# beilsme/rs-image-segmentation

Measured on AMD Instinct MI355X. Metric: Mpixel/s feature-extract+classify, higher is better.
Workload: dtype f32

## Files before the change

include/rsseg.h:

```cpp
#ifndef RSSEG_H
#define RSSEG_H

#include <stddef.h>
#include <stdint.h>

#ifdef __cplusplus
extern "C" {
#endif

#define RSSEG_OK 0
#define RSSEG_ERR_INVALID (-1)
#define RSSEG_ERR_HIP (-2)
#define RSSEG_ERR_NOMEM (-3)
#define RSSEG_ERR_COMM (-4)
#define RSSEG_ERR_UNSUPPORTED (-5)

#define RSSEG_F32 0
#define RSSEG_F64 1
#define RSSEG_I64 2
#define RSSEG_U8 3
#define RSSEG_I16 4
#define RSSEG_U16 5
#define RSSEG_I32 6

// ... 110 lines not shown
#define RSSEG_MORPH_GRADIENT 4
int rsseg_morph_u8(rsseg_ctx *ctx, const uint8_t *d_q, int H, int W, int k, int op, uint8_t *d_out);
int rsseg_morph_rows_u8(rsseg_ctx *ctx, const uint8_t *d_q, int Hin, int W, int y0, int y1, int edges, int k, int op,
                        uint8_t *d_out);
int rsseg_laplacian_norm_u8(rsseg_ctx *ctx, const uint8_t *d_q, int H, int W, float *d_out);
int rsseg_laplacian_norm_rows_u8(rsseg_ctx *ctx, const uint8_t *d_q, int Hin, int W, int y0, int y1, int edges, float *d_out);
int rsseg_sobel_mag_u8(rsseg_ctx *ctx, const uint8_t *d_q, int H, int W, float *d_out);
int rsseg_sobel_mag_rows_u8(rsseg_ctx *ctx, const uint8_t *d_q, int Hin, int W, int y0, int y1, int edges, float *d_out);

typedef struct rsseg_kmeans_info {
    int32_t n_iter;
    int32_t relocated;
    double tol;
    double scale[RSSEG_MAX_FEATURES];
    double min[RSSEG_MAX_FEATURES];
    double mean[RSSEG_MAX_FEATURES];
    int64_t init_indices[RSSEG_MAX_CLUSTERS];
    double ms_init;
    double ms_lloyd;
} rsseg_kmeans_info;

int rsseg_kmeans_fit_predict(rsseg_ctx *ctx, const void *const *d_planes, int F, int dtype, int64_t n_local,
                             int k, uint32_t seed, int max_iter, double tol, int32_t *d_labels,
                             double *centers, rsseg_kmeans_info *info);
int rsseg_kmeans_fit_predict_mm(rsseg_ctx *ctx, const void *const *d_planes, int F, int dtype, int64_t n_local, int k,
                                uint32_t seed, int max_iter, double tol, int32_t *d_labels, double *centers,
                                rsseg_kmeans_info *info, const double *local_min, const double *local_max);

int rsseg_forest_load(rsseg_ctx *ctx, int n_trees, const int64_t *tree_off, const int32_t *left,
                      const int32_t *right, const int32_t *feature, const double *threshold,
                      const uint8_t *missing_go_left, const double *value, int n_classes,
                      const int64_t *classes, int n_features);
int rsseg_forest_predict(rsseg_ctx *ctx, const float *const *d_planes, int F, int64_t n, int64_t *d_out);
int rsseg_forest_predict_proba(rsseg_ctx *ctx, const float *const *d_planes, int F, int64_t n, double *d_proba, double *d_conf,
                               int64_t *d_labels);
int rsseg_forest_oob(rsseg_ctx *ctx, const float *const *d_planes, int F, int64_t n, const int32_t *d_counts, double *d_oob,
                     int32_t *d_n_oob);

int rsseg_forest_fit(rsseg_ctx *ctx, const float *const *d_planes, int F, int64_t n, const int32_t *d_y, int n_classes,
                     const int32_t *d_counts, int same_counts, int n_trees, const uint32_t *seeds, int max_depth,
                     int min_samples_split, int min_samples_leaf, int max_features, const int64_t *node_off,
                     int32_t *d_left, int32_t *d_right, int32_t *d_feature, double *d_threshold, double *d_impurity,
                     int32_t *d_n_node, int32_t *d_w_node, uint8_t *d_missing_left, double *d_value,
                     int64_t *node_count, int32_t *max_depth_out);
typedef struct rsseg_forest_job {
    int64_t counts_row;
    int64_t weight_total;
    uint32_t seed;
    int32_t max_depth, min_samples_split, min_samples_leaf, max_features;
    int32_t reserved;
} rsseg_forest_job;
int rsseg_forest_fit_jobs(rsseg_ctx *ctx, const float *const *d_planes, int F, int64_t n, const int32_t *d_y, int n_classes,
                          const int32_t *d_counts, int64_t n_count_rows, int n_trees, const rsseg_forest_job *jobs,
                          const int64_t *node_off, int32_t *d_left, int32_t *d_right, int32_t *d_feature, double *d_threshold,
                          double *d_impurity, int32_t *d_n_node, int32_t *d_w_node, uint8_t *d_missing_left, double *d_value,
                          int64_t *node_count, int32_t *max_depth_out);

int rsseg_threshold_band_f32(rsseg_ctx *ctx, const float *d_x, int64_t n, float lo, float hi, uint8_t *d_out);
int rsseg_band_interval_f32(rsseg_ctx *ctx, const float *d_x, int64_t n, float lo, float hi, int nan_as_zero, uint8_t *d_out);
int rsseg_band_interval_f64(rsseg_ctx *ctx, const double *d_x, int64_t n, double lo, double hi, int nan_as_zero, uint8_t *d_out);
int rsseg_otsu_mask(rsseg_ctx *ctx, const void *d_x, int dtype, int64_t n, int above, uint8_t *d_out, int *level, double *vmin,
                    double *vmax);
int rsseg_mask_op_u8(rsseg_ctx *ctx, const uint8_t *d_a, const uint8_t *d_b, int64_t n, int op, uint8_t *d_out);
int rsseg_mask_paint_u8(rsseg_ctx *ctx, uint8_t *d_map, const uint8_t *d_mask, int64_t n, int value, int only_unset);
int rsseg_morph_ellipse_u8(rsseg_ctx *ctx, const uint8_t *d_q, int H, int W, int k, int op, uint8_t *d_out);
int rsseg_remove_small_components_u8(rsseg_ctx *ctx, const uint8_t *d_mask, int H, int W, int min_area, uint8_t *d_out);
// ... 23 lines not shown
```

rs-image-segmentation_amd/csrc/common.h:

```cpp
#pragma once
#include <hip/hip_runtime.h>
#include <stdint.h>
#include <stdio.h>
#include <string.h>

#include <map>
#include <string>
#include <vector>

#include "../../include/rsseg.h"

#define WAVE 64

struct prof_entry {
    double ms = 0.0;
    int64_t launches = 0;
    std::vector<std::pair<hipEvent_t, hipEvent_t>> pending;
};

struct forest_dev {
    void *d_nodes = nullptr;
    void *d_leafval = nullptr;
    void *d_treeoff = nullptr;
    void *d_groups = nullptr;
    int n_groups = 0;
    int n_trees = 0, n_classes = 0, n_features = 0, max_depth = 0;
    int64_t n_nodes = 0;
    int64_t classes[64];
};

struct rsseg_ctx {
    int device = 0;
    hipStream_t stream = nullptr;
    bool own_stream = false;
    bool async_mode = false;
    char err[512] = {0};
    int rank = 0, world = 1;
    std::vector<std::pair<const void *, int64_t>> byte_valued;
    bool comm_on = false;
    rsseg_allreduce_fn allreduce = nullptr;
    void *comm_user = nullptr;
    char *d_comm = nullptr;
    size_t comm_bytes = 0;
    char *h_comm = nullptr;
    void *rccl_comm = nullptr;
    bool own_comm_buf = false;
    char *d_ws = nullptr;
    size_t ws_bytes = 0;
    char *h_pin = nullptr;
    size_t pin_bytes = 0;
    bool prof_on = false;
    std::map<std::string, prof_entry> prof;
    std::vector<hipEvent_t> event_pool;
    forest_dev forest;
    bool mm_collect = false;
    uint32_t *d_mm = nullptr;
    int mm_count = 0;
// ... 196 lines not shown
```

rs-image-segmentation_amd/csrc/ctx.hip:

```cpp
#include <dlfcn.h>
#include <stdarg.h>

#include <chrono>
#include <mutex>

#include "common.h"

int rs_fail(rsseg_ctx *ctx, int code, const char *fmt, ...)
{
    if (ctx) {
        va_list ap;
        va_start(ap, fmt);
        vsnprintf(ctx->err, sizeof(ctx->err), fmt, ap);
        va_end(ap);
    }
    return code;
}

static thread_local char g_err[256] = "no context";

extern "C" const char *rsseg_version(void) { return "rsseg-hip 0.1 (gfx950)"; }

extern "C" const char *rsseg_last_error(const rsseg_ctx *ctx) { return ctx ? ctx->err : g_err; }

// ... 157 lines not shown
    ctx->world = world;
    ctx->allreduce = rccl_allreduce;
    ctx->comm_user = ctx;
    ctx->comm_on = true;
    if (hipHostMalloc((void **)&ctx->h_comm, comm_bytes, hipHostMallocDefault) != hipSuccess) {
        rccl_release(ctx);
        ctx->comm_on = false;
        ctx->allreduce = nullptr;
        return rs_fail(ctx, RSSEG_ERR_NOMEM, "hipHostMalloc(%zu) for the communication staging buffer failed", comm_bytes);
    }
    return RSSEG_OK;
}

extern "C" void rsseg_ctx_destroy(rsseg_ctx *ctx)
{
    if (!ctx) return;
    (void)hipSetDevice(ctx->device);
    (void)hipStreamSynchronize(ctx->stream);
    for (auto &kv : ctx->prof)
        for (auto &p : kv.second.pending) {
            (void)hipEventDestroy(p.first);
            (void)hipEventDestroy(p.second);
        }
    for (auto ev : ctx->event_pool) (void)hipEventDestroy(ev);
    if (ctx->d_ws) (void)hipFree(ctx->d_ws);
    if (ctx->h_pin) (void)hipHostFree(ctx->h_pin);
    if (ctx->h_comm) (void)hipHostFree(ctx->h_comm);
    rccl_release(ctx);
    if (ctx->d_mm) (void)hipFree(ctx->d_mm);
    if (ctx->forest.d_nodes) (void)hipFree(ctx->forest.d_nodes);
    if (ctx->forest.d_leafval) (void)hipFree(ctx->forest.d_leafval);
    if (ctx->forest.d_treeoff) (void)hipFree(ctx->forest.d_treeoff);
    if (ctx->forest.d_groups) (void)hipFree(ctx->forest.d_groups);
    if (ctx->own_stream) (void)hipStreamDestroy(ctx->stream);
    delete ctx;
}

extern "C" int rsseg_ctx_set_comm(rsseg_ctx *ctx, int rank, int world, rsseg_allreduce_fn fn, void *user,
                                  void *d_comm, size_t comm_bytes)
{
    if (!ctx) return RSSEG_ERR_INVALID;
    rccl_release(ctx);
    if (world < 1 || rank < 0 || rank >= world || world > RSSEG_MAX_RANKS)
        return rs_fail(ctx, RSSEG_ERR_INVALID, "bad rank/world %d/%d", rank, world);
    if (world > 1 && (!fn || !d_comm || comm_bytes < (1u << 20)))
        return rs_fail(ctx, RSSEG_ERR_INVALID, "world > 1 needs an all-reduce hook and a >= 1 MiB comm buffer");
    ctx->rank = rank;
    ctx->world = world;
    ctx->allreduce = fn;
    ctx->comm_user = user;
    ctx->d_comm = (char *)d_comm;
    ctx->comm_bytes = comm_bytes;
    ctx->comm_on = world > 1 || (fn && d_comm && comm_bytes >= (1u << 20));
    if (ctx->h_comm) (void)hipHostFree(ctx->h_comm);
    ctx->h_comm = nullptr;
    if (ctx->comm_on) {
        HIPCHK(ctx, hipSetDevice(ctx->device));
        if (hipHostMalloc((void **)&ctx->h_comm, comm_bytes, hipHostMallocDefault) != hipSuccess)
            return rs_fail(ctx, RSSEG_ERR_NOMEM, "hipHostMalloc(%zu) for the communication staging buffer failed", comm_bytes);
    }
    return RSSEG_OK;
}

static int comm_hook(rsseg_ctx *ctx, int64_t offset, int64_t count, int dtype, int op)
{
    const int rc = ctx->allreduce(ctx->comm_user, offset, count, dtype, op);
// ... 376 lines not shown
```

rs-image-segmentation_amd/csrc/k11_forest.h:

```cpp
#pragma once
#include <algorithm>

#include "common.h"

struct __align__(8) rf_node {
    float thr;
    unsigned bits;
};
#define RF_LEAF 0x00800000u
#define RF_MISS 0x00400000u
#define RF_CHILD 0x003fffffu
#define RF_NAN_BITS 0x7fc00000u
#define RF_PAY_MASK 0x003fffffu

#define RF_NCMAX 64
static_assert(RSSEG_MAX_FEATURES <= 64, "byte 3 of a node holds 4 * feature");
#define RF_C 4

struct rf_planes {
    const float *p[RSSEG_MAX_FEATURES];
};

struct rf_tree {
    int node_off;
// ... 6 lines not shown
    int first, count;
    int node_base;
    int n_nodes;
};

typedef __attribute__((address_space(3))) const float lds_cfloat;
typedef __attribute__((address_space(3))) const rf_node lds_cnode;
#if defined(__HIP_DEVICE_COMPILE__)
#define RF_LDS_PTR(T, a) ((T *)(a))
#else
#define RF_LDS_PTR(T, a) ((T *)(uintptr_t)(a))
#endif

template <int NC>
__device__ __forceinline__ void rf_row_load(const rf_node nd, const double *__restrict__ leafval, double (&row)[NC])
{
    const double2 *v = reinterpret_cast<const double2 *>(leafval + (size_t)(__float_as_uint(nd.thr) & RF_PAY_MASK) * NC);
#pragma unroll
    for (int c = 0; c < NC / 2; c++) {
        const double2 t = v[c];
        row[2 * c] = t.x;
        row[2 * c + 1] = t.y;
    }
}
template <int NC>
__device__ __forceinline__ void rf_vote(const rf_node nd, const double *__restrict__ leafval, double (&acc)[NC])
{
    double row[NC];
    rf_row_load<NC>(nd, leafval, row);
#pragma unroll
    for (int c = 0; c < NC; c++) acc[c] += row[c];
}


template <int TH>
__device__ __forceinline__ int rf_stage_features(const rf_planes &pl, int F, int64_t n, int64_t i, float *feat)
{
    int my_nan = 0;
    for (int f = 0; f < F; f++) {
        const float v = i < n ? pl.p[f][i] : 0.f;
        my_nan |= v != v;
        feat[f * TH + threadIdx.x] = v;
    }
    return my_nan;
}

#define RF_PX 1
#define RF_NCH (RF_PX * RF_C)

template <bool NANS>
__device__ __forceinline__ void rf_round_lds(rf_node (&nd)[RF_NCH], unsigned feat_tid, unsigned px_stride, const unsigned (&base)[RF_C])
{
    float x[RF_NCH];
#pragma unroll
    for (int q = 0; q < RF_NCH; q++)
        x[q] = *RF_LDS_PTR(lds_cfloat, feat_tid + (q / RF_C) * px_stride + (nd[q].bits >> 24));
#pragma unroll
    for (int q = 0; q < RF_NCH; q++) {
        bool go_right = x[q] > nd[q].thr;
        if (NANS) go_right = go_right || (x[q] != x[q] && !(nd[q].bits & RF_MISS));
        const unsigned next = (nd[q].bits & RF_CHILD) + (go_right ? 1u : 0u);
        lds_cnode *p = RF_LDS_PTR(lds_cnode, base[q % RF_C] + next * 8u);
        nd[q].thr = p->thr;
        nd[q].bits = p->bits;
    }
}
// ... 68 lines not shown
```

rs-image-segmentation_amd/csrc/k11_forest.hip:

```cpp
#include <algorithm>
#include <cmath>
#include <queue>

#include "common.h"
#include "k11_forest.h"

template <int NC>
__device__ __forceinline__ void rf_finish(const double (&acc)[NC], int n_trees, int n_classes, const long long *__restrict__ classes,
                                          long long *__restrict__ out, int64_t i)
{
    int best = 0;
    double bv = acc[0] / (double)n_trees;
#pragma unroll
    for (int c = 1; c < NC; c++)
        if (c < n_classes) {
            const double p = acc[c] / (double)n_trees;
            if (p > bv) { bv = p; best = c; }
        }
    out[i] = classes[best];
}

template <int NC, int RF_TH>
__global__ __launch_bounds__(RF_TH) void k11_forest_lds(rf_planes pl, int F, int64_t n, const rf_node *__restrict__ nodes,
                                                        const rf_tree *__restrict__ trees, const rf_group *__restrict__ groups, int n_groups,
                                                        int cap2 , int two_rounds, int n_trees,
                                                        const double *__restrict__ leafval,
                                                        int n_classes, const long long *__restrict__ classes, long long *__restrict__ out)
{
    constexpr int RF_LT = RF_TH / RF_PX;
    extern __shared__ __align__(16) char smem[];
    const int FP = F | 1;
    float *feat = reinterpret_cast<float *>(smem);
    uint4 *top = reinterpret_cast<uint4 *>(feat + (size_t)FP * RF_TH);
    const int64_t i0 = (int64_t)blockIdx.x * RF_TH + threadIdx.x;
    int my_nan = 0;
    for (int f = 0; f < F; f++)
#pragma unroll
        for (int p = 0; p < RF_PX; p++) {
            const int64_t i = i0 + p * RF_LT;
            const float v = i < n ? pl.p[f][i] : 0.f;
            my_nan |= v != v;
            feat[(p * RF_LT + threadIdx.x) * FP + f] = v;
        }
    {
        const rf_group g0 = groups[0];
        const uint4 *src = reinterpret_cast<const uint4 *>(nodes + g0.node_base);
        for (int j = threadIdx.x; j < (g0.n_nodes + 1) / 2; j += RF_LT) top[j] = src[j];
        if (threadIdx.x == 0) top[cap2] = make_uint4(RF_NAN_BITS, RF_LEAF | RF_MISS, RF_NAN_BITS, RF_LEAF | RF_MISS);
    }
    const bool any_nan = __syncthreads_or(my_nan) != 0;
    const unsigned feat_tid = (unsigned)(uintptr_t)(lds_cfloat *)feat + threadIdx.x * (unsigned)FP * 4u;
    const unsigned px_stride = (unsigned)RF_LT * (unsigned)FP * 4u;
    const unsigned top_addr = (unsigned)(uintptr_t)(__attribute__((address_space(3))) const uint4 *)top;
    double acc[RF_PX][NC];
#pragma unroll
    for (int p = 0; p < RF_PX; p++)
#pragma unroll
        for (int c = 0; c < NC; c++) acc[p][c] = 0.0;
    for (int g = 0; g < n_groups; g++) {
        const rf_group gr = groups[g];
        static_assert(RF_NPRE == 6, "the prefetch registers below are spelled out for six pieces per thread");
        const bool more = g + 1 < n_groups;
        const rf_group gn = groups[more ? g + 1 : g];
        const int npiece = more ? (gn.n_nodes + 1) / 2 : 0;
        const uint4 *psrc = reinterpret_cast<const uint4 *>(nodes + gn.node_base);
        const int plast = (gn.n_nodes + 1) / 2 - 1;
#define RF_PRE(r) const uint4 pre##r = psrc[(int)threadIdx.x + r * RF_LT < plast ? (int)threadIdx.x + r * RF_LT : plast];
        RF_PRE(0) RF_PRE(1) RF_PRE(2) RF_PRE(3) RF_PRE(4) RF_PRE(5)
#undef RF_PRE
        rf_node nd[RF_NCH];
        unsigned base[RF_C];
#pragma unroll
        for (int c = 0; c < RF_C; c++) {
            const rf_tree tr = trees[c < gr.count ? gr.first + c : gr.first];
            base[c] = c < gr.count ? top_addr + (unsigned)(tr.node_off - gr.node_base) * 8u : top_addr + (unsigned)cap2 * 16u;
            lds_cnode *p = RF_LDS_PTR(lds_cnode, base[c]);
#pragma unroll
            for (int px = 0; px < RF_PX; px++) {
                nd[px * RF_C + c].thr = p->thr;
                nd[px * RF_C + c].bits = p->bits;
            }
        }
        if (any_nan) rf_walk_lds<true>(nd, feat_tid, px_stride, base, two_rounds != 0);
        else rf_walk_lds<false>(nd, feat_tid, px_stride, base, two_rounds != 0);
        constexpr bool PIPE = NC <= 8;
        double rows[PIPE ? RF_NCH : 1][NC];
        if (PIPE) {
#pragma unroll
            for (int q = 0; q < RF_NCH; q++) rf_row_load<NC>(nd[q], leafval, rows[PIPE ? q : 0]);
        } else {
#pragma unroll
            for (int q = 0; q < RF_NCH; q++)
                if (q % RF_C < gr.count && i0 + (q / RF_C) * RF_LT < n) rf_vote<NC>(nd[q], leafval, acc[q / RF_C]);
        }
        if (more) {
            __syncthreads();
#define RF_PUT(r) if ((int)threadIdx.x + r * RF_LT < npiece) top[threadIdx.x + r * RF_LT] = pre##r;
            RF_PUT(0) RF_PUT(1) RF_PUT(2) RF_PUT(3) RF_PUT(4) RF_PUT(5)
#undef RF_PUT
        }
        if (more) __syncthreads();
        if (PIPE) {
#pragma unroll
            for (int q = 0; q < RF_NCH; q++)
                if (q % RF_C < gr.count) {
#pragma unroll
                    for (int c = 0; c < NC; c++) acc[q / RF_C][c] += rows[PIPE ? q : 0][c];
                }
        }
    }
#pragma unroll
    for (int px = 0; px < RF_PX; px++)
        if (i0 + px * RF_LT < n) rf_finish<NC>(acc[px], n_trees, n_classes, classes, out, i0 + px * RF_LT);
}

template <int NC, int RF_TH>
__global__ __launch_bounds__(RF_TH) void k11_forest_gen(rf_planes pl, int F, int64_t n, const rf_node *__restrict__ nodes,
                                                        const rf_tree *__restrict__ trees, int n_trees, int ntop,
                                                        const double *__restrict__ leafval, int n_classes,
                                                        const long long *__restrict__ classes, long long *__restrict__ out)
{
    extern __shared__ __align__(16) char smem[];
    float *feat = reinterpret_cast<float *>(smem);
    rf_node *top = reinterpret_cast<rf_node *>(feat + (size_t)F * RF_TH);
    const int64_t i = (int64_t)blockIdx.x * RF_TH + threadIdx.x;
    const int my_nan = rf_stage_features<RF_TH>(pl, F, n, i, feat);
    constexpr int NPRE = 12;
    for (int c = 0; c < RF_C && c < n_trees; c++) {
        const rf_tree t0 = trees[c];
        const int cnt = t0.n_nodes < ntop ? t0.n_nodes : ntop;
        for (int j = threadIdx.x; j < cnt; j += RF_TH) top[(size_t)c * ntop + j] = nodes[t0.node_off + j];
    }
    const bool any_nan = __syncthreads_or(my_nan) != 0;
    double acc[NC];
#pragma unroll
    for (int c = 0; c < NC; c++) acc[c] = 0.0;
    const int n_groups = (n_trees + RF_C - 1) / RF_C;
    for (int g = 0; g < n_groups; g++) {
        const int t = g * RF_C;
        rf_tree tr[RF_C];
#pragma unroll
        for (int c = 0; c < RF_C; c++) tr[c] = trees[t + c < n_trees ? t + c : n_trees - 1];
        rf_node pre[NPRE];
        int pcnt[RF_C], poff[RF_C];
        const bool more = t + RF_C < n_trees;
        if (more) {
// ... 134 lines not shown
                const unsigned tb = RF_NAN_BITS | pay;
                memcpy(&nd.thr, &tb, 4);
                nd.bits = RF_LEAF | RF_MISS | (unsigned)h;
            } else {
                const bool swap = std::isnan(threshold[g]);
                float f = swap ? INFINITY : (float)threshold[g];
                if (!swap && (double)f > threshold[g]) f = nextafterf(f, -INFINITY);
                nd.thr = f;
                const bool miss_left = missing_go_left && missing_go_left[g];
                const int first = swap ? right[g] : left[g], second = swap ? left[g] : right[g];
                nd.bits = (unsigned)newid[first] | ((unsigned)feature[g] << 26) | ((miss_left != swap) ? RF_MISS : 0u);
                if (newid[second] != newid[first] + 1) return rs_fail(ctx, RSSEG_ERR_INVALID, "forest_load: internal layout error");
            }
        }
    }
    const int cap = rf_lds_cap(n_features, rf_threads(n_features, n_classes));
    std::vector<rf_group> groups;
    bool fits = true;
    for (int t = 0; t < n_trees && fits;) {
        rf_group g;
        g.first = t;
        g.node_base = trees[t].node_off & ~1;
        g.count = 0;
        g.n_nodes = 0;
        while (t < n_trees && g.count < RF_C && trees[t].node_off + trees[t].n_nodes - g.node_base <= cap) {
            g.n_nodes = trees[t].node_off + trees[t].n_nodes - g.node_base;
            g.count++;
            t++;
        }
        if (g.count == 0) fits = false;
        else groups.push_back(g);
    }
    if (!fits) groups.clear();
    forest_dev &fd = ctx->forest;
    HIPCHK(ctx, rs_sync(ctx));
    if (fd.d_nodes) HIPCHK(ctx, hipFree(fd.d_nodes));
    if (fd.d_leafval) HIPCHK(ctx, hipFree(fd.d_leafval));
    if (fd.d_treeoff) HIPCHK(ctx, hipFree(fd.d_treeoff));
    if (fd.d_groups) HIPCHK(ctx, hipFree(fd.d_groups));
    fd.d_nodes = fd.d_leafval = fd.d_treeoff = fd.d_groups = nullptr;
    fd.n_groups = (int)groups.size();
    if (!groups.empty()) {
        HIPCHK(ctx, hipMalloc(&fd.d_groups, groups.size() * sizeof(rf_group)));
        HIPCHK(ctx, hipMemcpy(fd.d_groups, groups.data(), groups.size() * sizeof(rf_group), hipMemcpyHostToDevice));
    }
    HIPCHK(ctx, hipMalloc(&fd.d_nodes, nodes.size() * sizeof(rf_node) + 64));
    HIPCHK(ctx, hipMalloc(&fd.d_leafval, leaf.size() * sizeof(double) + 64));
    HIPCHK(ctx, hipMalloc(&fd.d_treeoff, n_classes * sizeof(long long) + trees.size() * sizeof(rf_tree) + 64));
    HIPCHK(ctx, hipMemcpy(fd.d_nodes, nodes.data(), nodes.size() * sizeof(rf_node), hipMemcpyHostToDevice));
    HIPCHK(ctx, hipMemcpy(fd.d_leafval, leaf.data(), leaf.size() * sizeof(double), hipMemcpyHostToDevice));
    HIPCHK(ctx, hipMemcpy(fd.d_treeoff, classes, n_classes * sizeof(long long), hipMemcpyHostToDevice));
    HIPCHK(ctx, hipMemcpy((char *)fd.d_treeoff + n_classes * sizeof(long long), trees.data(), trees.size() * sizeof(rf_tree), hipMemcpyHostToDevice));
    fd.n_trees = n_trees;
    fd.max_depth = max_depth;
    fd.n_classes = n_classes;
    fd.n_features = n_features;
    fd.n_nodes = nn;
    for (int c = 0; c < n_classes; c++) fd.classes[c] = classes[c];
    return RSSEG_OK;
}

extern "C" int rsseg_forest_predict(rsseg_ctx *ctx, const float *const *d_planes, int F, int64_t n, int64_t *d_out)
{
    if (!ctx) return RSSEG_ERR_INVALID;
    forest_dev &fd = ctx->forest;
    if (!fd.d_nodes) return rs_fail(ctx, RSSEG_ERR_INVALID, "forest_predict: no forest loaded");
    if (!d_planes || !d_out || n < 0) return rs_fail(ctx, RSSEG_ERR_INVALID, "forest_predict: bad arguments");
    if (F != fd.n_features)
        return rs_fail(ctx, RSSEG_ERR_INVALID, "forest_predict: X has %d features, but the forest is expecting %d features as input", F, fd.n_features);
    HIPCHK(ctx, hipSetDevice(ctx->device));
    rf_planes pl;
    memset(&pl, 0, sizeof(pl));
    for (int f = 0; f < F; f++) {
        if (!d_planes[f]) return rs_fail(ctx, RSSEG_ERR_INVALID, "forest_predict: plane %d is null", f);
        pl.p[f] = d_planes[f];
    }
    if (n == 0) return RSSEG_OK;
    const long long *d_classes = (const long long *)fd.d_treeoff;
    const rf_tree *d_trees = (const rf_tree *)((const char *)fd.d_treeoff + fd.n_classes * sizeof(long long));
    const int TH = rf_threads(F, fd.n_classes);
    const unsigned grid = (unsigned)ceil_div64(n, TH);
    int rc;
    if (fd.n_groups > 0) {
        const int cap = rf_lds_cap(F, TH);
        const size_t lds = (size_t)(F | 1) * TH * 4 + (size_t)cap * sizeof(rf_node) + 16;
        auto launch = [&](auto kern) -> int {
            RSCHK(set_max_dyn_lds(ctx, (const void *)kern, lds));
            prof_scope ps(ctx, "forest");
            hipLaunchKernelGGL(kern, dim3(grid), dim3(TH / RF_PX), lds, ctx->stream, pl, F, n, (const rf_node *)fd.d_nodes, d_trees,
                               (const rf_group *)fd.d_groups, fd.n_groups, cap / 2, fd.max_depth >= 10 ? 1 : 0, fd.n_trees, (const double *)fd.d_leafval, fd.n_classes, d_classes,
                               (long long *)d_out);
            return RSSEG_OK;
        };
        if (TH == 1024) {
            if (fd.n_classes <= 4) rc = launch(k11_forest_lds<4, 1024>);
            else if (fd.n_classes <= 8) rc = launch(k11_forest_lds<8, 1024>);
            else if (fd.n_classes <= 16) rc = launch(k11_forest_lds<16, 1024>);
            else rc = launch(k11_forest_lds<32, 1024>);
        } else {
            if (fd.n_classes <= 4) rc = launch(k11_forest_lds<4, 512>);
            else if (fd.n_classes <= 8) rc = launch(k11_forest_lds<8, 512>);
            else if (fd.n_classes <= 16) rc = launch(k11_forest_lds<16, 512>);
            else if (fd.n_classes <= 32) rc = launch(k11_forest_lds<32, 512>);
            else rc = launch(k11_forest_lds<64, 512>);
        }
    } else {
        int ntop = 3 * TH;
        while (ntop > 256 && (size_t)F * TH * 4 + (size_t)RF_C * ntop * sizeof(rf_node) > 158 * 1024) ntop -= 256;
        const size_t lds = (size_t)F * TH * 4 + (size_t)RF_C * ntop * sizeof(rf_node);
        auto launch = [&](auto kern) -> int {
            RSCHK(set_max_dyn_lds(ctx, (const void *)kern, lds));
            prof_scope ps(ctx, "forest");
            hipLaunchKernelGGL(kern, dim3(grid), dim3(TH), lds, ctx->stream, pl, F, n, (const rf_node *)fd.d_nodes, d_trees, fd.n_trees, ntop,
                               (const double *)fd.d_leafval, fd.n_classes, d_classes, (long long *)d_out);
            return RSSEG_OK;
        };
        if (TH == 1024) {
            if (fd.n_classes <= 4) rc = launch(k11_forest_gen<4, 1024>);
            else if (fd.n_classes <= 8) rc = launch(k11_forest_gen<8, 1024>);
            else if (fd.n_classes <= 16) rc = launch(k11_forest_gen<16, 1024>);
            else rc = launch(k11_forest_gen<32, 1024>);
        } else {
            if (fd.n_classes <= 4) rc = launch(k11_forest_gen<4, 512>);
            else if (fd.n_classes <= 8) rc = launch(k11_forest_gen<8, 512>);
            else if (fd.n_classes <= 16) rc = launch(k11_forest_gen<16, 512>);
            else if (fd.n_classes <= 32) rc = launch(k11_forest_gen<32, 512>);
            else rc = launch(k11_forest_gen<64, 512>);
        }
    }
    if (rc != RSSEG_OK) return rc;
    HIPCHK(ctx, hipGetLastError());
    return stream_sync(ctx);
}
```

rs-image-segmentation_amd/rsseg/_lib.py:

```python
from __future__ import annotations

import ctypes as C
import os

_HERE = os.path.dirname(os.path.abspath(__file__))
LIB_PATH = os.path.join(os.path.dirname(_HERE), "librsseg_hip.so")

MAX_FEATURES = 64
MAX_CLUSTERS = 64
MAX_RANKS = 16
F32, F64, I64 = 0, 1, 2
U8, I16, U16, I32 = 3, 4, 5, 6
EVAL_MAX_CELLS = 4096
SUM, MIN, MAX = 0, 1, 2
BORDER_REFLECT, BORDER_REFLECT101 = 0, 1
MORPH_ERODE, MORPH_DILATE, MORPH_OPEN, MORPH_CLOSE, MORPH_GRADIENT = 0, 1, 2, 3, 4
MASK_AND, MASK_OR, MASK_ANDNOT, MASK_NOT = 0, 1, 2, 3

ALLREDUCE_FN = C.CFUNCTYPE(C.c_int, C.c_void_p, C.c_int64, C.c_int64, C.c_int, C.c_int)


class KMeansInfo(C.Structure):
    _fields_ = [
        ("n_iter", C.c_int32),
# ... 57 lines not shown
    "rsseg_glcm_u8": (_int, [_vp, _vp, _int, _int, _int, _int, _int, _PP]),
    "rsseg_glcm_offsets_u8": (_int, [_vp, _vp, _int, _int, _int, _int, _int, C.POINTER(C.c_int32), _int, _PP]),
    "rsseg_quantize_u8": (_int, [_vp, _vp, _i64, C.c_float, _vp]),
    "rsseg_u8_to_unit_f32": (_int, [_vp, _vp, _i64, _vp]),
    "rsseg_u8_to_f32": (_int, [_vp, _vp, _i64, _vp]),
    "rsseg_resize_bilinear_f32": (_int, [_vp, _vp, _int, _int, _vp, _int, _int]),
    "rsseg_resize_bilinear_rows_f32": (_int, [_vp, _vp, _int, _int, _int, _int, _vp, _int, _int, _int, _int]),
    "rsseg_resize_bilinear_rows_multi_f32": (_int, [_vp, _PP, _int, _int, _int, _int, _int, _PP, _int, _int, _int, _int]),
    "rsseg_box_mean_f32": (_int, [_vp, _vp, _int, _int, _int, _int, _int, _vp]),
    "rsseg_box_mean_rows_f32": (_int, [_vp, _PP, _int, _int, _int, _int, _int, _int, _int, _int, _int, _PP]),
    "rsseg_local_std_rows_f32": (_int, [_vp, _vp, _int, _int, _int, _int, _int, _int, _int, _vp]),
    "rsseg_morph_rows_u8": (_int, [_vp, _vp, _int, _int, _int, _int, _int, _int, _int, _vp]),
    "rsseg_laplacian_norm_rows_u8": (_int, [_vp, _vp, _int, _int, _int, _int, _int, _vp]),
    "rsseg_sobel_mag_rows_u8": (_int, [_vp, _vp, _int, _int, _int, _int, _int, _vp]),
    "rsseg_local_std_f32": (_int, [_vp, _vp, _int, _int, _int, _vp]),
    "rsseg_morph_gradient_u8": (_int, [_vp, _vp, _int, _int, _int, _vp]),
    "rsseg_morph_u8": (_int, [_vp, _vp, _int, _int, _int, _int, _vp]),
    "rsseg_local_var_f32": (_int, [_vp, _vp, _int, _int, _int, _vp]),
    "rsseg_laplacian_norm_u8": (_int, [_vp, _vp, _int, _int, _vp]),
    "rsseg_sobel_mag_u8": (_int, [_vp, _vp, _int, _int, _vp]),
    "rsseg_kmeans_fit_predict": (_int, [_vp, _PP, _int, _int, _i64, _int, C.c_uint32, _int, C.c_double, _vp,
                                        C.POINTER(C.c_double), C.POINTER(KMeansInfo)]),
    "rsseg_kmeans_fit_predict_mm": (_int, [_vp, _PP, _int, _int, _i64, _int, C.c_uint32, _int, C.c_double, _vp,
                                           C.POINTER(C.c_double), C.POINTER(KMeansInfo), C.POINTER(C.c_double), C.POINTER(C.c_double)]),
    "rsseg_ctx_allreduce": (_int, [_vp, _i64, _i64, _int, _int]),
    "rsseg_rccl_unique_id": (_int, [C.c_char_p, _vp]),
    "rsseg_ctx_set_comm_rccl": (_int, [_vp, _int, _int, _vp, C.c_char_p, _vp, C.c_size_t]),
    "rsseg_ctx_collect_minmax": (_int, [_vp, _int]),
    "rsseg_ctx_last_minmax": (_int, [_vp, _int, C.POINTER(C.c_double), C.POINTER(C.c_double)]),
    "rsseg_forest_load": (_int, [_vp, _int, C.POINTER(_i64), C.POINTER(C.c_int32), C.POINTER(C.c_int32),
                                 C.POINTER(C.c_int32), C.POINTER(C.c_double), C.POINTER(C.c_uint8),
                                 C.POINTER(C.c_double), _int, C.POINTER(_i64), _int]),
    "rsseg_forest_predict": (_int, [_vp, _PP, _int, _i64, _vp]),
    "rsseg_forest_predict_proba": (_int, [_vp, _PP, _int, _i64, _vp, _vp, _vp]),
    "rsseg_forest_oob": (_int, [_vp, _PP, _int, _i64, _vp, _vp, _vp]),
    "rsseg_forest_fit": (_int, [_vp, _PP, _int, _i64, _vp, _int, _vp, _int, _int, C.POINTER(C.c_uint32), _int, _int, _int, _int,
                                C.POINTER(_i64), _vp, _vp, _vp, _vp, _vp, _vp, _vp, _vp, _vp, C.POINTER(_i64),
                                C.POINTER(C.c_int32)]),
    "rsseg_forest_fit_jobs": (_int, [_vp, _PP, _int, _i64, _vp, _int, _vp, _i64, _int, _vp, C.POINTER(_i64), _vp, _vp, _vp, _vp, _vp, _vp, _vp,
                                     _vp, _vp, C.POINTER(_i64), C.POINTER(C.c_int32)]),
    "rsseg_threshold_band_f32": (_int, [_vp, _vp, _i64, C.c_float, C.c_float, _vp]),
    "rsseg_band_interval_f32": (_int, [_vp, _vp, _i64, C.c_float, C.c_float, _int, _vp]),
    "rsseg_band_interval_f64": (_int, [_vp, _vp, _i64, C.c_double, C.c_double, _int, _vp]),
    "rsseg_otsu_mask": (_int, [_vp, _vp, _int, _i64, _int, _vp, C.POINTER(_int), C.POINTER(C.c_double), C.POINTER(C.c_double)]),
    "rsseg_fill_holes_u8": (_int, [_vp, _vp, _int, _int, _vp]),
    "rsseg_mask_op_u8": (_int, [_vp, _vp, _vp, _i64, _int, _vp]),
    "rsseg_mask_paint_u8": (_int, [_vp, _vp, _vp, _i64, _int, _int]),
    "rsseg_morph_ellipse_u8": (_int, [_vp, _vp, _int, _int, _int, _int, _vp]),
    "rsseg_remove_small_components_u8": (_int, [_vp, _vp, _int, _int, _int, _vp]),
    "rsseg_lbp_uniform_u8": (_int, [_vp, _vp, _int, _int, _int, C.c_double, _vp]),
    "rsseg_rank_entropy_u8": (_int, [_vp, _vp, _int, _int, _int, _vp]),
    "rsseg_gaussian_blur_u8": (_int, [_vp, _vp, _int, _int, _int, _vp]),
    "rsseg_confusion_counts": (_int, [_vp, _vp, _int, _vp, _int, _i64, C.POINTER(_i64), C.POINTER(_i64), C.POINTER(_i64),
                                      C.POINTER(_i64), _i64]),
    "rsseg_preprocess_u8": (_int, [_vp, _PP, _int, _int, _i64, C.POINTER(C.c_double), C.POINTER(C.c_double), _PP,
                                   C.POINTER(C.c_double)]),
    "rsseg_radiometric": (_int, [_vp, _vp, _int, _i64, C.c_double, C.c_double, _vp]),
    "rsseg_host_gaussian_kernel_fixed": (_int, [_int, C.POINTER(_int)]),
    "rsseg_host_lzw_encode": (_i64, [_vp, _i64, _vp, _i64]),
    "rsseg_host_lzw_decode": (_i64, [_vp, _i64, _vp, _i64]),
    "rsseg_host_kmeans_draws": (_int, [C.c_uint32, _i64, _int, _int, C.POINTER(_i64), C.POINTER(C.c_double)]),
}

_lib = None


# ... 23 lines not shown
```

rs-image-segmentation_amd/rsseg/runtime.py:

```python
from __future__ import annotations

import ctypes as C
import os
from typing import List, Optional, Sequence, Tuple

import numpy as np

from . import _lib as L


class RssegError(RuntimeError):
    pass


class RssegUnsupported(RssegError):
    """RSSEG_ERR_UNSUPPORTED: a valid input beyond a capacity of the kernels (more than 64 features / classes, ...).
    Never swallowed by the mirrors: the reference would have produced a result, so an all-zero map would be a lie."""


def _torch():
    import torch
    return torch


# ... 580 lines not shown
            self._chk(self.lib.rsseg_kmeans_fit_predict_mm(self.h, self._pp(planes), F, L.F32, n, n_clusters, seed, max_iter, tol,
                                                           C.c_void_p(labels.data_ptr()), centers.ctypes.data_as(C.POINTER(C.c_double)),
                                                           C.byref(info), lmin, lmax))
        else:
            self._chk(self.lib.rsseg_kmeans_fit_predict(self.h, self._pp(planes), F, L.F32 if dt == torch.float32 else L.F64, n,
                                                        n_clusters, seed, max_iter, tol, C.c_void_p(labels.data_ptr()),
                                                        centers.ctypes.data_as(C.POINTER(C.c_double)), C.byref(info)))
        meta = dict(n_iter=info.n_iter, tol=info.tol, relocated=info.relocated,
                    scale=np.array(info.scale[:F]), min=np.array(info.min[:F]), mean=np.array(info.mean[:F]),
                    init_indices=np.array(info.init_indices[:n_clusters]), ms_init=info.ms_init, ms_lloyd=info.ms_lloyd,
                    centers=centers)
        return labels[:n], meta

    def forest_load(self, forest: dict):
        f = forest
        ip, lp, dp = C.POINTER(C.c_int32), C.POINTER(C.c_int64), C.POINTER(C.c_double)
        keep = [np.ascontiguousarray(f["tree_off"], np.int64), np.ascontiguousarray(f["left"], np.int32),
                np.ascontiguousarray(f["right"], np.int32), np.ascontiguousarray(f["feature"], np.int32),
                np.ascontiguousarray(f["threshold"], np.float64), np.ascontiguousarray(f["missing_left"], np.uint8),
                np.ascontiguousarray(f["value"], np.float64), np.ascontiguousarray(f["classes"], np.int64)]
        self._chk(self.lib.rsseg_forest_load(self.h, len(keep[0]) - 1, keep[0].ctypes.data_as(lp), keep[1].ctypes.data_as(ip),
                                             keep[2].ctypes.data_as(ip), keep[3].ctypes.data_as(ip), keep[4].ctypes.data_as(dp),
                                             keep[5].ctypes.data_as(C.POINTER(C.c_uint8)), keep[6].ctypes.data_as(dp),
                                             keep[6].shape[1], keep[7].ctypes.data_as(lp), int(f["n_features"])))
        self._forest_shape = (len(keep[0]) - 1, int(keep[6].shape[1]), int(f["n_features"]))

    def forest_predict(self, planes: Sequence):
        torch = _torch()
        n = planes[0].numel()
        out = self.empty(n, torch.int64)
        self._chk(self.lib.rsseg_forest_predict(self.h, self._pp(planes), len(planes), n, C.c_void_p(out.data_ptr())))
        return out

    def forest_predict_proba(self, planes: Sequence, proba: bool = True, confidence: bool = False, labels: bool = False):
        torch = _torch()
        n = planes[0].numel()
        nc = getattr(self, "_forest_shape", (0, 1, 0))[1]
        p = self.empty(nc * n, torch.float64) if proba else None
        c = self.empty(n, torch.float64) if confidence else None
        lab = self.empty(n, torch.int64) if labels else None
        ptr = lambda t: None if t is None else C.c_void_p(t.data_ptr())
        self._chk(self.lib.rsseg_forest_predict_proba(self.h, self._pp(planes), len(planes), n, ptr(p), ptr(c), ptr(lab)))
        return (None if p is None else p.view(nc, n)), c, lab

    def forest_oob(self, planes: Sequence, counts):
        torch = _torch()
        n = planes[0].numel()
        nt, nc, _ = getattr(self, "_forest_shape", (0, 1, 0))
        if counts is not None and (counts.dtype != torch.int32 or counts.numel() != nt * n or not counts.is_contiguous()):
            raise ValueError(f"forest_oob: counts must be {nt} x {n} contiguous int32 values (one row per tree of the loaded forest)")
        oob = self.empty(nc * n, torch.float64)
        n_oob = self.empty(n, torch.int32)
        self._chk(self.lib.rsseg_forest_oob(self.h, self._pp(planes), len(planes), n, None if counts is None else C.c_void_p(counts.data_ptr()),
                                            C.c_void_p(oob.data_ptr()), C.c_void_p(n_oob.data_ptr())))
        return oob.view(nc, n), n_oob

    def forest_fit(self, planes: Sequence, y, counts, seeds: np.ndarray, node_caps: np.ndarray, max_depth: int,
                   min_samples_split: int, min_samples_leaf: int, max_features: int, n_classes: int) -> List[dict]:
        same = counts.numel() == planes[0].numel()
        seeds = np.ascontiguousarray(seeds, np.uint32)
        vp = lambda t: C.c_void_p(t.data_ptr())

        def call(n, off, out, nc, md):
            return self.lib.rsseg_forest_fit(self.h, self._pp(planes), len(planes), n, vp(y), int(n_classes), vp(counts), int(same), len(seeds),
                                             seeds.ctypes.data_as(C.POINTER(C.c_uint32)), int(max_depth), int(min_samples_split),
                                             int(min_samples_leaf), int(max_features), off, *out, nc, md)
# ... 149 lines not shown
```

Before: 3791.

## Certify forest votes with 16-bit integer leaf tables and re-run only uncertain pixels

Adds a first forest-predict pass that accumulates 16-bit quantized leaf probabilities in integer registers. It writes the label directly wherever the top-two vote margin exceeds the worst-case quantization error. Uncertain pixels are appended to a device list through a wave-aggregated atomic, and a second exact double-precision pass walks only those listed pixels; blocks beyond the list size exit early. The goal is to shrink leaf-table traffic and replace f64 accumulation, at the cost of an extra launch, a memset and a full exact rerun if the list capacity overflows. A stats query and a profiling script are also added.

```diff
diff --git a/include/rsseg.h b/include/rsseg.h
--- a/include/rsseg.h
+++ b/include/rsseg.h
@@ -166,6 +166,7 @@
                       const uint8_t *missing_go_left, const double *value, int n_classes,
                       const int64_t *classes, int n_features);
 int rsseg_forest_predict(rsseg_ctx *ctx, const float *const *d_planes, int F, int64_t n, int64_t *d_out);
+int rsseg_forest_vote_stats(rsseg_ctx *ctx, long long out[3]);
 int rsseg_forest_predict_proba(rsseg_ctx *ctx, const float *const *d_planes, int F, int64_t n, double *d_proba, double *d_conf,
                                int64_t *d_labels);
 int rsseg_forest_oob(rsseg_ctx *ctx, const float *const *d_planes, int F, int64_t n, const int32_t *d_counts, double *d_oob,
diff --git a/profiles/forest_votes_stats.py b/profiles/forest_votes_stats.py
--- /dev/null
+++ b/profiles/forest_votes_stats.py
@@ -0,0 +1,39 @@
+import json
+import os
+import sys
+import time
+
+ROOT = os.path.dirname(os.path.dirname(os.path.abspath(__file__)))
+for p in (os.path.join(ROOT, "rs-image-segmentation_amd"), ROOT):
+    sys.path.insert(0, p)
+import numpy as np
+import torch
+
+import bench as B
+from rsseg import pipeline as P
+from rsseg.runtime import Context
+
+size = int(sys.argv[1]) if len(sys.argv) > 1 else 16384
+reps = int(sys.argv[2]) if len(sys.argv) > 2 else 3
+dev = torch.device("cuda", 0)
+ctx = Context(0, use_dist=False)
+fm = B.fit_c5_forest(torch, None, dev, P, 0, 1, 16384)
+ctx.forest_load(fm["flat"])
+H = W = size
+bands = B.synth_rows(torch, dev, W, 0, H)
+planes, _ = P.feature_stack19(ctx, bands, H, W)
+fp = P.stack19_forest_planes(ctx, planes)
+out = ctx.forest_predict(fp)
+torch.cuda.synchronize()
+t0 = time.perf_counter()
+for _ in range(reps):
+    out = ctx.forest_predict(fp)
+torch.cuda.synchronize()
+ms = (time.perf_counter() - t0) / reps * 1e3
+st = ctx.forest_vote_stats()
+idx = np.random.default_rng(0).choice(H * W, 20000, replace=False)
+ti = torch.from_numpy(idx).to(dev)
+X = np.stack([p[ti].cpu().numpy() for p in fp], 1)
+mism = int((fm["model"].predict(X) != out[ti].cpu().numpy()).sum())
+print(json.dumps(dict(size=size, pixels=H * W, forest_ms=round(ms, 2), votes=os.environ.get("RSSEG_FOREST_VOTES", "certified"), **st,
+                      listed_share=st["listed"] / (H * W), list_capacity=H * W // 64 + 1024, sklearn_mismatch_of_20000=mism)), flush=True)
diff --git a/rs-image-segmentation_amd/csrc/common.h b/rs-image-segmentation_amd/csrc/common.h
--- a/rs-image-segmentation_amd/csrc/common.h
+++ b/rs-image-segmentation_amd/csrc/common.h
@@ -23,6 +23,10 @@
     void *d_leafval = nullptr;
     void *d_treeoff = nullptr;
     void *d_groups = nullptr;
+    void *d_leafq = nullptr;
+    void *d_vote_count = nullptr;
+    int vote_cert = 0;
+    long long vote_cap = 0;
     int n_groups = 0;
     int n_trees = 0, n_classes = 0, n_features = 0, max_depth = 0;
     int64_t n_nodes = 0;
diff --git a/rs-image-segmentation_amd/csrc/ctx.hip b/rs-image-segmentation_amd/csrc/ctx.hip
--- a/rs-image-segmentation_amd/csrc/ctx.hip
+++ b/rs-image-segmentation_amd/csrc/ctx.hip
@@ -213,6 +213,8 @@
     if (ctx->forest.d_leafval) (void)hipFree(ctx->forest.d_leafval);
     if (ctx->forest.d_treeoff) (void)hipFree(ctx->forest.d_treeoff);
     if (ctx->forest.d_groups) (void)hipFree(ctx->forest.d_groups);
+    if (ctx->forest.d_leafq) (void)hipFree(ctx->forest.d_leafq);
+    if (ctx->forest.d_vote_count) (void)hipFree(ctx->forest.d_vote_count);
     if (ctx->own_stream) (void)hipStreamDestroy(ctx->stream);
     delete ctx;
 }
diff --git a/rs-image-segmentation_amd/csrc/k11_forest.h b/rs-image-segmentation_amd/csrc/k11_forest.h
--- a/rs-image-segmentation_amd/csrc/k11_forest.h
+++ b/rs-image-segmentation_amd/csrc/k11_forest.h
@@ -62,6 +62,64 @@
     for (int c = 0; c < NC; c++) acc[c] += row[c];
 }
 
+#define RF_VOTEQ_ONE 32768.0
+#define RF_VOTEQ_MAX_TREES 65535
+
+template <int NC>
+__device__ __forceinline__ void rf_rowq_load(const rf_node nd, const unsigned short *__restrict__ leafq, unsigned (&row)[NC / 2])
+{
+    const unsigned short *r = leafq + (size_t)(__float_as_uint(nd.thr) & RF_PAY_MASK) * NC;
+    if constexpr (NC == 4) {
+        const uint2 t = *reinterpret_cast<const uint2 *>(r);
+        row[0] = t.x;
+        row[1] = t.y;
+    } else {
+        const uint4 *v = reinterpret_cast<const uint4 *>(r);
+#pragma unroll
+        for (int c = 0; c < NC / 8; c++) {
+            const uint4 t = v[c];
+            row[4 * c] = t.x;
+            row[4 * c + 1] = t.y;
+            row[4 * c + 2] = t.z;
+            row[4 * c + 3] = t.w;
+        }
+    }
+}
+template <int NC>
+__device__ __forceinline__ void rf_rowq_add(const unsigned (&row)[NC / 2], unsigned (&acc)[NC])
+{
+#pragma unroll
+    for (int c = 0; c < NC / 2; c++) {
+        acc[2 * c] += row[c] & 0xffffu;
+        acc[2 * c + 1] += row[c] >> 16;
+    }
+}
+template <int NC, bool CERT>
+struct rf_votes;
+template <int NC>
+struct rf_votes<NC, false> {
+    typedef double acc_t;
+    typedef double table_t;
+    static constexpr int ROW = NC;
+    typedef double row_t;
+    static constexpr bool PIPE = NC <= 8;
+    static __device__ __forceinline__ void load(const rf_node nd, const table_t *__restrict__ t, row_t (&row)[ROW]) { rf_row_load<NC>(nd, t, row); }
+    static __device__ __forceinline__ void add(const row_t (&row)[ROW], acc_t (&acc)[NC])
+    {
+#pragma unroll
+        for (int c = 0; c < NC; c++) acc[c] += row[c];
+    }
+};
+template <int NC>
+struct rf_votes<NC, true> {
+    typedef unsigned acc_t;
+    typedef unsigned short table_t;
+    static constexpr int ROW = NC / 2;
+    typedef unsigned row_t;
+    static constexpr bool PIPE = NC <= 16;
+    static __device__ __forceinline__ void load(const rf_node nd, const table_t *__restrict__ t, row_t (&row)[ROW]) { rf_rowq_load<NC>(nd, t, row); }
+    static __device__ __forceinline__ void add(const row_t (&row)[ROW], acc_t (&acc)[NC]) { rf_rowq_add<NC>(row, acc); }
+};
 
 template <int TH>
 __device__ __forceinline__ int rf_stage_features(const rf_planes &pl, int F, int64_t n, int64_t i, float *feat)
diff --git a/rs-image-segmentation_amd/csrc/k11_forest.hip b/rs-image-segmentation_amd/csrc/k11_forest.hip
--- a/rs-image-segmentation_amd/csrc/k11_forest.hip
+++ b/rs-image-segmentation_amd/csrc/k11_forest.hip
@@ -20,19 +20,43 @@
     out[i] = classes[best];
 }
 
-template <int NC, int RF_TH>
+template <int NC>
+__device__ __forceinline__ bool rf_finish_cert(const unsigned (&acc)[NC], int n_trees, int &best)
+{
+    unsigned b = acc[0], s = 0;
+    best = 0;
+#pragma unroll
+    for (int c = 1; c < NC; c++) {
+        const unsigned v = acc[c];
+        s = v > b ? b : (v > s ? v : s);
+        if (v > b) { b = v; best = c; }
+    }
+    return b - s > (unsigned)n_trees + 2u;
+}
+
+template <int NC, int RF_TH, bool CERT>
 __global__ __launch_bounds__(RF_TH) void k11_forest_lds(rf_planes pl, int F, int64_t n, const rf_node *__restrict__ nodes,
                                                         const rf_tree *__restrict__ trees, const rf_group *__restrict__ groups, int n_groups,
                                                         int cap2 , int two_rounds, int n_trees,
-                                                        const double *__restrict__ leafval,
-                                                        int n_classes, const long long *__restrict__ classes, long long *__restrict__ out)
-{
+                                                        const typename rf_votes<NC, CERT>::table_t *__restrict__ leafval,
+                                                        int n_classes, const long long *__restrict__ classes, long long *__restrict__ out,
+                                                        long long *list, unsigned long long *count, long long list_cap)
+{
+    typedef rf_votes<NC, CERT> votes;
     constexpr int RF_LT = RF_TH / RF_PX;
     extern __shared__ __align__(16) char smem[];
     const int FP = F | 1;
     float *feat = reinterpret_cast<float *>(smem);
     uint4 *top = reinterpret_cast<uint4 *>(feat + (size_t)FP * RF_TH);
-    const int64_t i0 = (int64_t)blockIdx.x * RF_TH + threadIdx.x;
+    int64_t i0 = (int64_t)blockIdx.x * RF_TH + threadIdx.x;
+    if (!CERT && list) {
+        static_assert(RF_PX == 1, "a listed pixel is the thread's only pixel");
+        const long long cnt = (long long)*count;
+        if (cnt <= list_cap) {
+            if ((long long)blockIdx.x * RF_TH >= cnt) return;
+            i0 = i0 < cnt ? list[i0] : n;
+        }
+    }
     int my_nan = 0;
     for (int f = 0; f < F; f++)
 #pragma unroll
@@ -52,11 +76,11 @@
     const unsigned feat_tid = (unsigned)(uintptr_t)(lds_cfloat *)feat + threadIdx.x * (unsigned)FP * 4u;
     const unsigned px_stride = (unsigned)RF_LT * (unsigned)FP * 4u;
     const unsigned top_addr = (unsigned)(uintptr_t)(__attribute__((address_space(3))) const uint4 *)top;
-    double acc[RF_PX][NC];
+    typename votes::acc_t acc[RF_PX][NC];
 #pragma unroll
     for (int p = 0; p < RF_PX; p++)
 #pragma unroll
-        for (int c = 0; c < NC; c++) acc[p][c] = 0.0;
+        for (int c = 0; c < NC; c++) acc[p][c] = 0;
     for (int g = 0; g < n_groups; g++) {
         const rf_group gr = groups[g];
         static_assert(RF_NPRE == 6, "the prefetch registers below are spelled out for six pieces per thread");
@@ -83,15 +107,18 @@
         }
         if (any_nan) rf_walk_lds<true>(nd, feat_tid, px_stride, base, two_rounds != 0);
         else rf_walk_lds<false>(nd, feat_tid, px_stride, base, two_rounds != 0);
-        constexpr bool PIPE = NC <= 8;
-        double rows[PIPE ? RF_NCH : 1][NC];
+        constexpr bool PIPE = votes::PIPE;
+        typename votes::row_t rows[PIPE ? RF_NCH : 1][votes::ROW];
         if (PIPE) {
 #pragma unroll
-            for (int q = 0; q < RF_NCH; q++) rf_row_load<NC>(nd[q], leafval, rows[PIPE ? q : 0]);
+            for (int q = 0; q < RF_NCH; q++) votes::load(nd[q], leafval, rows[PIPE ? q : 0]);
         } else {
 #pragma unroll
             for (int q = 0; q < RF_NCH; q++)
-                if (q % RF_C < gr.count && i0 + (q / RF_C) * RF_LT < n) rf_vote<NC>(nd[q], leafval, acc[q / RF_C]);
+                if (q % RF_C < gr.count && i0 + (q / RF_C) * RF_LT < n) {
+                    votes::load(nd[q], leafval, rows[0]);
+                    votes::add(rows[0], acc[q / RF_C]);
+                }
         }
         if (more) {
             __syncthreads();
@@ -103,15 +130,31 @@
         if (PIPE) {
 #pragma unroll
             for (int q = 0; q < RF_NCH; q++)
-                if (q % RF_C < gr.count) {
-#pragma unroll
-                    for (int c = 0; c < NC; c++) acc[q / RF_C][c] += rows[PIPE ? q : 0][c];
-                }
-        }
-    }
-#pragma unroll
-    for (int px = 0; px < RF_PX; px++)
-        if (i0 + px * RF_LT < n) rf_finish<NC>(acc[px], n_trees, n_classes, classes, out, i0 + px * RF_LT);
+                if (q % RF_C < gr.count) votes::add(rows[PIPE ? q : 0], acc[q / RF_C]);
+        }
+    }
+    if constexpr (!CERT) {
+#pragma unroll
+        for (int px = 0; px < RF_PX; px++)
+            if (i0 + px * RF_LT < n) rf_finish<NC>(acc[px], n_trees, n_classes, classes, out, i0 + px * RF_LT);
+    } else {
+#pragma unroll
+        for (int px = 0; px < RF_PX; px++) {
+            const int64_t i = i0 + px * RF_LT;
+            int best;
+            const bool sure = rf_finish_cert<NC>(acc[px], n_trees, best);
+            if (i < n && sure) out[i] = classes[best];
+            const bool open = i < n && !sure;
+            const unsigned long long m = __ballot(open);
+            if (m) {
+                const int lane = lane_id(), leader = __ffsll((long long)m) - 1;
+                unsigned long long at = 0;
+                if (lane == leader) at = atomicAdd(count, (unsigned long long)__popcll(m));
+                at = __shfl(at, leader, 64) + (unsigned long long)__popcll(m & ((1ull << lane) - 1ull));
+                if (open && (long long)at < list_cap) list[at] = i;
+            }
+        }
+    }
 }
 
 template <int NC, int RF_TH>
@@ -312,13 +355,24 @@
         else groups.push_back(g);
     }
     if (!fits) groups.clear();
+    std::vector<unsigned short> leafq;
+    if (!groups.empty() && n_trees <= RF_VOTEQ_MAX_TREES) {
+        leafq.resize(leaf.size());
+        for (size_t j = 0; j < leaf.size(); j++) {
+            const double v = leaf[j];
+            if (!(v >= 0.0 && v <= 1.0)) { leafq.clear(); break; }
+            leafq[j] = (unsigned short)std::floor(v * RF_VOTEQ_ONE + 0.5);
+        }
+    }
     forest_dev &fd = ctx->forest;
     HIPCHK(ctx, rs_sync(ctx));
     if (fd.d_nodes) HIPCHK(ctx, hipFree(fd.d_nodes));
     if (fd.d_leafval) HIPCHK(ctx, hipFree(fd.d_leafval));
     if (fd.d_treeoff) HIPCHK(ctx, hipFree(fd.d_treeoff));
     if (fd.d_groups) HIPCHK(ctx, hipFree(fd.d_groups));
-    fd.d_nodes = fd.d_leafval = fd.d_treeoff = fd.d_groups = nullptr;
+    if (fd.d_leafq) HIPCHK(ctx, hipFree(fd.d_leafq));
+    fd.d_nodes = fd.d_leafval = fd.d_treeoff = fd.d_groups = fd.d_leafq = nullptr;
+    fd.vote_cert = 0;
     fd.n_groups = (int)groups.size();
     if (!groups.empty()) {
         HIPCHK(ctx, hipMalloc(&fd.d_groups, groups.size() * sizeof(rf_group)));
@@ -329,6 +383,11 @@
     HIPCHK(ctx, hipMalloc(&fd.d_treeoff, n_classes * sizeof(long long) + trees.size() * sizeof(rf_tree) + 64));
     HIPCHK(ctx, hipMemcpy(fd.d_nodes, nodes.data(), nodes.size() * sizeof(rf_node), hipMemcpyHostToDevice));
     HIPCHK(ctx, hipMemcpy(fd.d_leafval, leaf.data(), leaf.size() * sizeof(double), hipMemcpyHostToDevice));
+    if (!leafq.empty()) {
+        HIPCHK(ctx, hipMalloc(&fd.d_leafq, leafq.size() * sizeof(unsigned short) + 64));
+        HIPCHK(ctx, hipMemcpy(fd.d_leafq, leafq.data(), leafq.size() * sizeof(unsigned short), hipMemcpyHostToDevice));
+        if (!fd.d_vote_count) HIPCHK(ctx, hipMalloc(&fd.d_vote_count, sizeof(unsigned long long)));
+    }
     HIPCHK(ctx, hipMemcpy(fd.d_treeoff, classes, n_classes * sizeof(long long), hipMemcpyHostToDevice));
     HIPCHK(ctx, hipMemcpy((char *)fd.d_treeoff + n_classes * sizeof(long long), trees.data(), trees.size() * sizeof(rf_tree), hipMemcpyHostToDevice));
     fd.n_trees = n_trees;
@@ -356,6 +415,7 @@
         pl.p[f] = d_planes[f];
     }
     if (n == 0) return RSSEG_OK;
+    fd.vote_cert = 0;
     const long long *d_classes = (const long long *)fd.d_treeoff;
     const rf_tree *d_trees = (const rf_tree *)((const char *)fd.d_treeoff + fd.n_classes * sizeof(long long));
     const int TH = rf_threads(F, fd.n_classes);
@@ -364,25 +424,49 @@
     if (fd.n_groups > 0) {
         const int cap = rf_lds_cap(F, TH);
         const size_t lds = (size_t)(F | 1) * TH * 4 + (size_t)cap * sizeof(rf_node) + 16;
-        auto launch = [&](auto kern) -> int {
-            RSCHK(set_max_dyn_lds(ctx, (const void *)kern, lds));
+        const char *mode = getenv("RSSEG_FOREST_VOTES");
+        const bool cert = fd.d_leafq && !(mode && !strcmp(mode, "exact"));
+        const long long list_cap = cert ? (long long)(n / 64 + 1024) : 0;
+        long long *d_list = nullptr;
+        unsigned long long *d_count = nullptr;
+        if (cert) {
+            RSCHK(ws_reserve(ctx, (size_t)list_cap * sizeof(long long)));
+            d_list = (long long *)ctx->d_ws;
+            d_count = (unsigned long long *)fd.d_vote_count;
+        }
+        auto launch = [&](auto kcert, auto kexact) -> int {
+            RSCHK(set_max_dyn_lds(ctx, (const void *)kexact, lds));
+            if (cert) {
+                RSCHK(set_max_dyn_lds(ctx, (const void *)kcert, lds));
+                HIPCHK(ctx, hipMemsetAsync(d_count, 0, sizeof(unsigned long long), ctx->stream));
+            }
             prof_scope ps(ctx, "forest");
-            hipLaunchKernelGGL(kern, dim3(grid), dim3(TH / RF_PX), lds, ctx->stream, pl, F, n, (const rf_node *)fd.d_nodes, d_trees,
+            if (cert)
+                hipLaunchKernelGGL(kcert, dim3(grid), dim3(TH / RF_PX), lds, ctx->stream, pl, F, n, (const rf_node *)fd.d_nodes, d_trees,
+                                   (const rf_group *)fd.d_groups, fd.n_groups, cap / 2, fd.max_depth >= 10 ? 1 : 0, fd.n_trees,
+                                   (const unsigned short *)fd.d_leafq, fd.n_classes, d_classes, (long long *)d_out, d_list, d_count, list_cap);
+            hipLaunchKernelGGL(kexact, dim3(grid), dim3(TH / RF_PX), lds, ctx->stream, pl, F, n, (const rf_node *)fd.d_nodes, d_trees,
                                (const rf_group *)fd.d_groups, fd.n_groups, cap / 2, fd.max_depth >= 10 ? 1 : 0, fd.n_trees, (const double *)fd.d_leafval, fd.n_classes, d_classes,
-                               (long long *)d_out);
+                               (long long *)d_out, d_list, d_count, list_cap);
             return RSSEG_OK;
         };
+#define RF_LAUNCH(NC, T) launch(k11_forest_lds<NC, T, true>, k11_forest_lds<NC, T, false>)
         if (TH == 1024) {
-            if (fd.n_classes <= 4) rc = launch(k11_forest_lds<4, 1024>);
-            else if (fd.n_classes <= 8) rc = launch(k11_forest_lds<8, 1024>);
-            else if (fd.n_classes <= 16) rc = launch(k11_forest_lds<16, 1024>);
-            else rc = launch(k11_forest_lds<32, 1024>);
+            if (fd.n_classes <= 4) rc = RF_LAUNCH(4, 1024);
+            else if (fd.n_classes <= 8) rc = RF_LAUNCH(8, 1024);
+            else if (fd.n_classes <= 16) rc = RF_LAUNCH(16, 1024);
+            else rc = RF_LAUNCH(32, 1024);
         } else {
-            if (fd.n_classes <= 4) rc = launch(k11_forest_lds<4, 512>);
-            else if (fd.n_classes <= 8) rc = launch(k11_forest_lds<8, 512>);
-            else if (fd.n_classes <= 16) rc = launch(k11_forest_lds<16, 512>);
-            else if (fd.n_classes <= 32) rc = launch(k11_forest_lds<32, 512>);
-            else rc = launch(k11_forest_lds<64, 512>);
+            if (fd.n_classes <= 4) rc = RF_LAUNCH(4, 512);
+            else if (fd.n_classes <= 8) rc = RF_LAUNCH(8, 512);
+            else if (fd.n_classes <= 16) rc = RF_LAUNCH(16, 512);
+            else if (fd.n_classes <= 32) rc = RF_LAUNCH(32, 512);
+            else rc = RF_LAUNCH(64, 512);
+        }
+#undef RF_LAUNCH
+        if (rc == RSSEG_OK) {
+            fd.vote_cert = cert ? 1 : 0;
+            fd.vote_cap = list_cap;
         }
     } else {
         int ntop = 3 * TH;
@@ -412,3 +496,20 @@
     HIPCHK(ctx, hipGetLastError());
     return stream_sync(ctx);
 }
+
+extern "C" int rsseg_forest_vote_stats(rsseg_ctx *ctx, long long out[3])
+{
+    if (!ctx) return RSSEG_ERR_INVALID;
+    if (!out) return rs_fail(ctx, RSSEG_ERR_INVALID, "forest_vote_stats: null argument");
+    forest_dev &fd = ctx->forest;
+    out[0] = out[1] = out[2] = 0;
+    if (!fd.vote_cert || !fd.d_vote_count) return RSSEG_OK;
+    HIPCHK(ctx, hipSetDevice(ctx->device));
+    unsigned long long cnt = 0;
+    HIPCHK(ctx, rs_sync(ctx));
+    HIPCHK(ctx, hipMemcpy(&cnt, fd.d_vote_count, sizeof(cnt), hipMemcpyDeviceToHost));
+    out[0] = 1;
+    out[1] = (long long)cnt;
+    out[2] = (long long)cnt > fd.vote_cap ? 1 : 0;
+    return RSSEG_OK;
+}
diff --git a/rs-image-segmentation_amd/rsseg/_lib.py b/rs-image-segmentation_amd/rsseg/_lib.py
--- a/rs-image-segmentation_amd/rsseg/_lib.py
+++ b/rs-image-segmentation_amd/rsseg/_lib.py
@@ -113,6 +113,7 @@
                                  C.POINTER(C.c_int32), C.POINTER(C.c_double), C.POINTER(C.c_uint8),
                                  C.POINTER(C.c_double), _int, C.POINTER(_i64), _int]),
     "rsseg_forest_predict": (_int, [_vp, _PP, _int, _i64, _vp]),
+    "rsseg_forest_vote_stats": (_int, [_vp, C.POINTER(C.c_longlong)]),
     "rsseg_forest_predict_proba": (_int, [_vp, _PP, _int, _i64, _vp, _vp, _vp]),
     "rsseg_forest_oob": (_int, [_vp, _PP, _int, _i64, _vp, _vp, _vp]),
     "rsseg_forest_fit": (_int, [_vp, _PP, _int, _i64, _vp, _int, _vp, _int, _int, C.POINTER(C.c_uint32), _int, _int, _int, _int,
diff --git a/rs-image-segmentation_amd/rsseg/runtime.py b/rs-image-segmentation_amd/rsseg/runtime.py
--- a/rs-image-segmentation_amd/rsseg/runtime.py
+++ b/rs-image-segmentation_amd/rsseg/runtime.py
@@ -636,6 +636,11 @@
         self._chk(self.lib.rsseg_forest_predict(self.h, self._pp(planes), len(planes), n, C.c_void_p(out.data_ptr())))
         return out
 
+    def forest_vote_stats(self) -> dict:
+        out = (C.c_longlong * 3)()
+        self._chk(self.lib.rsseg_forest_vote_stats(self.h, out))
+        return dict(certified=bool(out[0]), listed=int(out[1]), overflow=bool(out[2]))
+
     def forest_predict_proba(self, planes: Sequence, proba: bool = True, confidence: bool = False, labels: bool = False):
         torch = _torch()
         n = planes[0].numel()
```

Result: no change. 3776 (-0.4%).
